# stefanvanberkum/gcnn-cut-selector

Hardware: AMD Instinct MI355X
Metric: bipartite-graph edges/sec (fwd+bwd) per training step, setcov-500 batch=32 (higher is better)
Workload: dtype f32; 1 GPU; setcov-500 rows x batch 32 per GPU (BASELINE configs[1]); step=fwd + mse + bwd + adam, launch=eager, problem=setcov, batch_per_gpu=32, global_batch=32, n_cons=16000, n_vars=32000, n_cuts=1893, n_cons_edges=800000, n_cut_edges=199704, parallelism=dp1

## Files before the change

### gcnn-cut-selector_amd/csrc/k_rows.hpp

```cpp
#pragma once
#include "gcnn_common.hpp"

__device__ __forceinline__ f32x4 mfma16(float a, float b, f32x4 c) {
    return __builtin_amdgcn_mfma_f32_16x16x4f32(a, b, c, 0, 0, 0);
}

struct RTile { float v[4][4]; };

__device__ __forceinline__ const float* lds_here(const float* p) {
    int zero = 0;
    asm volatile("" : "+v"(zero));
    return p + zero;
}

__device__ __forceinline__ void rt_zero(RTile& t) {
#pragma unroll
    for (int m = 0; m < 4; ++m)
#pragma unroll
        for (int i = 0; i < 4; ++i) t.v[m][i] = 0.f;
}
__device__ __forceinline__ void rt_load(RTile& t, const float* x, int row, bool ok, int g) {
#pragma unroll
    for (int m = 0; m < 4; ++m) {
        float4 f = make_float4(0.f, 0.f, 0.f, 0.f);
        if (ok) f = *(const float4*)(x + (size_t)row * EMB + 16 * m + 4 * g);
        t.v[m][0] = f.x; t.v[m][1] = f.y; t.v[m][2] = f.z; t.v[m][3] = f.w;
    }
}
template <int ST = ST_PLAIN>
__device__ __forceinline__ void rt_store(const RTile& t, float* x, int row, bool ok, int g) {
    if (!ok || !x) return;
#pragma unroll
    for (int m = 0; m < 4; ++m) store16<ST>(x + (size_t)row * EMB + 16 * m + 4 * g, t.v[m][0], t.v[m][1], t.v[m][2], t.v[m][3]);
}
enum { GEMM_FWD = 0, GEMM_BWD = 1, GEMM_FWD_RM = 2 };
template <int MODE>
__device__ __forceinline__ void rt_gemm(const RTile& t, float scale, const float* wl, f32x4 (&acc)[4], int lane) {
    const int m = lane & 15, g = lane >> 4;
    wl = lds_here(wl);
#pragma unroll
    for (int mt = 0; mt < 4; ++mt) {
        float av[4][4];
        if (MODE == GEMM_BWD) {
#pragma unroll
            for (int mo = 0; mo < 4; ++mo) {
                const float4 w4 = *(const float4*)(wl + (16 * mo + m) * LDW + 16 * mt + 4 * g);
                av[mo][0] = w4.x; av[mo][1] = w4.y; av[mo][2] = w4.z; av[mo][3] = w4.w;
            }
        } else if (MODE == GEMM_FWD) {
// ... 51 lines not shown
            const float v = o.v[m][i] + bv[i];
            o.v[m][i] = RELU ? fmaxf(v, 0.f) : v;
        }
    }
}
__device__ __forceinline__ void rt_mask(RTile& o, const RTile& act) {
#pragma unroll
    for (int m = 0; m < 4; ++m)
#pragma unroll
        for (int i = 0; i < 4; ++i) o.v[m][i] = act.v[m][i] > 0.f ? o.v[m][i] : 0.f;
}
typedef unsigned short mask16;
__device__ __forceinline__ unsigned rt_mask_bits(const RTile& t) {
    unsigned b = 0;
#pragma unroll
    for (int m = 0; m < 4; ++m)
#pragma unroll
        for (int i = 0; i < 4; ++i) b |= (t.v[m][i] > 0.f ? 1u : 0u) << (4 * m + i);
    return b;
}
__device__ __forceinline__ void rt_mask_store(const RTile& t, mask16* dst, int row, bool ok, int g) {
    if (ok && dst) dst[(size_t)row * 4 + g] = (mask16)rt_mask_bits(t);
}
__device__ __forceinline__ unsigned rt_mask_load(const mask16* src, int row, bool ok, int g) {
    return ok ? (unsigned)src[(size_t)row * 4 + g] : 0u;
}
__device__ __forceinline__ void rt_mask_apply(RTile& o, unsigned bits) {
#pragma unroll
    for (int m = 0; m < 4; ++m)
#pragma unroll
        for (int i = 0; i < 4; ++i) o.v[m][i] = (bits >> (4 * m + i)) & 1u ? o.v[m][i] : 0.f;
}
__device__ __forceinline__ void rt_clear_unless(RTile& o, bool ok) {
#pragma unroll
    for (int m = 0; m < 4; ++m)
#pragma unroll
        for (int i = 0; i < 4; ++i) o.v[m][i] = ok ? o.v[m][i] : 0.f;
}

template <int NM, int NV, int NT, bool K4 = false>
__device__ __forceinline__ void stage_lds(float* smem, const float* const (&w)[NM], const float* const (&v)[NV]) {
    constexpr int PER = 1024 / NT;
    float4 tmp[NM][PER];
    float vec[NV];
    if (K4) {
#pragma unroll
        for (int wi = 0; wi < NM; ++wi)
#pragma unroll
// ... 22 lines not shown
                *(float4*)(smem + wi * 64 * LDW + (idx >> 4) * LDW + (idx & 15) * 4) = tmp[wi][i];
            }
        }
    if (threadIdx.x < 64) {
#pragma unroll
        for (int vi = 0; vi < NV; ++vi) smem[NM * 64 * LDW + vi * 64 + threadIdx.x] = vec[vi];
    }
}
#define ROWS_LDS_FLOATS(NM, NV) ((NM) * 64 * LDW + (NV) * 64)

struct EmbArgs {
    const float *x, *shift, *scale, *w1, *b1; mask16* m_e1;
    const float *w2, *b2; float* xo; mask16* m_x;
    const float* wp[2]; const float* bp[2]; float* po[2];
    int n;
};
template <int F, int NPROJ, int NT, int ST = ST_PLAIN>
__device__ __forceinline__ void emb_program(const EmbArgs& a, float* smem, int bid, int nblk) {
    constexpr int NWAVES = NT / 64, NM = 1 + NPROJ, NV = 2 + NPROJ;
    const int lane = threadIdx.x & 63, wv = threadIdx.x >> 6, j = lane & 15, g = lane >> 4;
    const int ntile = (a.n + 15) >> 4;
    float* vecs = smem + NM * 64 * LDW;
    float* w1s = smem + ROWS_LDS_FLOATS(NM, NV);
    int tile = bid + nblk * wv;
    float xv[F], xn_[F];
    auto load_ops = [&](float (&dst)[F], int t) {
        const int row = t * 16 + j;
#pragma unroll
        for (int f = 0; f < F; ++f) dst[f] = row < a.n ? a.x[(size_t)row * F + f] : 0.f;
    };
    load_ops(xv, tile);
    constexpr int W1N = (F * 64 + NT - 1) / NT;
    float w1r[W1N];
#pragma unroll
    for (int q = 0; q < W1N; ++q) { const int i = threadIdx.x + q * NT; w1r[q] = i < F * 64 ? a.w1[i] : 0.f; }
    if (NPROJ == 2) {
        const float* const w[3] = {a.w2, a.wp[0], a.wp[1]};
        const float* const v[4] = {a.b1, a.b2, a.bp[0], a.bp[1]};
        stage_lds<3, 4, NT, true>((float*)smem, w, v);
    } else {
        const float* const w[2] = {a.w2, a.wp[0]};
        const float* const v[3] = {a.b1, a.b2, a.bp[0]};
        stage_lds<2, 3, NT, true>((float*)smem, w, v);
    }
#pragma unroll
    for (int q = 0; q < W1N; ++q) { const int i = threadIdx.x + q * NT; if (i < F * 64) w1s[i] = w1r[q]; }
    float shift[F], scale[F];
#pragma unroll
    for (int f = 0; f < F; ++f) { shift[f] = a.shift[f]; scale[f] = a.scale[f]; }
    __syncthreads();
    for (; tile < ntile; tile += nblk * NWAVES) {
        load_ops(xn_, tile + nblk * NWAVES);
        const int row = tile * 16 + j;
        const bool ok = row < a.n;
        RTile o, t;
        rt_zero(o);
        const float* w1h = lds_here(w1s);
#pragma unroll
        for (int f = 0; f < F; ++f) {
            const float xn = ok ? (xv[f] + shift[f]) * scale[f] : 0.f;
#pragma unroll
            for (int m = 0; m < 4; ++m) {
                const float4 w = *(const float4*)(w1h + f * EMB + 16 * m + 4 * g);
                o.v[m][0] = fmaf(xn, w.x, o.v[m][0]); o.v[m][1] = fmaf(xn, w.y, o.v[m][1]);
                o.v[m][2] = fmaf(xn, w.z, o.v[m][2]); o.v[m][3] = fmaf(xn, w.w, o.v[m][3]);
            }
        }
        rt_bias<true>(o, vecs, g);
        rt_clear_unless(o, ok);
        rt_mask_store(o, a.m_e1, row, ok, g);
        rt_mm<false>(t, o, 1.f, smem, lane);
        rt_bias<true>(t, vecs + 64, g);
        rt_clear_unless(t, ok);
        rt_store<ST>(t, a.xo, row, ok, g);
        rt_mask_store(t, a.m_x, row, ok, g);
#pragma unroll
        for (int k = 0; k < NPROJ; ++k) {
            rt_mm<false>(o, t, 1.f, smem + (1 + k) * 64 * LDW, lane);
            rt_bias<false>(o, vecs + (2 + k) * 64, g);
            rt_store<ST>(o, a.po[k], row, ok, g);
        }
#pragma unroll
        for (int f = 0; f < F; ++f) xv[f] = xn_[f];
    }
}
#define FUSE_WF (EMB * EMB + EMB)
#define FUSE_W1A (FUSE_WF + EMB * EMB)
#define FUSE_BF (FUSE_W1A + EMB * EMB)
#define FUSE_FLOATS (FUSE_BF + EMB)
struct FuseArgs { const float *wf[3], *bf[3], *s2[3], *w1a[3]; float* out[3]; };
__device__ __forceinline__ void fuse_weights(const FuseArgs& f, const int k, float* smem) {
    float* wfs = smem;
    float* was = smem + 64 * LDW;
    const int t = threadIdx.x;
    if (t < 256) {
        for (int q = t; q < 1024; q += 256) {
            const float4 a = *(const float4*)(f.wf[k] + q * 4), b = *(const float4*)(f.w1a[k] + q * 4);
            *(float4*)(wfs + (q >> 4) * LDW + (q & 15) * 4) = a;
            *(float4*)(was + (q >> 4) * LDW + (q & 15) * 4) = b;
            *(float4*)(f.out[k] + FUSE_WF + q * 4) = a;
            *(float4*)(f.out[k] + FUSE_W1A + q * 4) = b;
        }
        if (t < EMB) f.out[k][FUSE_BF + t] = f.bf[k][t];
    }
    __syncthreads();
    if (t >= 256) return;
// ... 49 lines not shown
    const float* targets; float loss_scale; float* g_o1; float* head_partial;
    int n;
};
enum { CF_PROJ = 0, CF_READOUT = 1, CF_LOSS = 2 };
#define HEAD_SLAB (2 * EMB)
__device__ __forceinline__ float row_sum16(float x) {
    x += __builtin_bit_cast(float, __builtin_amdgcn_update_dpp(0, __builtin_bit_cast(int, x), 0x121, 0xf, 0xf, false));
    x += __builtin_bit_cast(float, __builtin_amdgcn_update_dpp(0, __builtin_bit_cast(int, x), 0x122, 0xf, 0xf, false));
    x += __builtin_bit_cast(float, __builtin_amdgcn_update_dpp(0, __builtin_bit_cast(int, x), 0x124, 0xf, 0xf, false));
    x += __builtin_bit_cast(float, __builtin_amdgcn_update_dpp(0, __builtin_bit_cast(int, x), 0x128, 0xf, 0xf, false));
    return x;
}
__device__ __forceinline__ float readout_score(const RTile& o1, const float* ws_lds, float bs, int g) {
    float sum = 0.f;
    const float* wsv = lds_here(ws_lds);
#pragma unroll
    for (int m = 0; m < 4; ++m) {
        const float4 w = *(const float4*)(wsv + 16 * m + 4 * g);
        sum = fmaf(o1.v[m][0], w.x, fmaf(o1.v[m][1], w.y, fmaf(o1.v[m][2], w.z, fmaf(o1.v[m][3], w.w, sum))));
    }
    sum += __shfl_xor(sum, 16); sum += __shfl_xor(sum, 32);
    return sum + bs;
}
__device__ __forceinline__ void loss_head_tile(RTile& go, const RTile& o1, float score, const ConvFArgs& a, const float* ws_lds,
                                               int tile, int row, bool ok, int lane) {
    const int j = lane & 15, g = lane >> 4;
    const float dlt = ok ? score - a.targets[row] : 0.f;
    const float ds = 2.f * dlt * a.loss_scale;
    const float* wsv = lds_here(ws_lds);
    float* slab = a.head_partial + (size_t)tile * HEAD_SLAB;
#pragma unroll
    for (int m = 0; m < 4; ++m) {
        const float4 w = *(const float4*)(wsv + 16 * m + 4 * g);
        const float wv4[4] = {w.x, w.y, w.z, w.w};
        float cs[4];
#pragma unroll
        for (int i = 0; i < 4; ++i) {
            go.v[m][i] = o1.v[m][i] > 0.f ? ds * wv4[i] : 0.f;
            cs[i] = row_sum16(ds * o1.v[m][i]);
        }
        if (j == 0) *(float4*)(slab + 16 * m + 4 * g) = make_float4(cs[0], cs[1], cs[2], cs[3]);
    }
    const float dbs = row_sum16(ds), ls = row_sum16(a.loss_scale * dlt * dlt);
    if (lane == 0) { slab[EMB] = dbs; slab[EMB + 1] = ls; }
}
template <int TAIL, int NT, bool KEEP_A = false, int ST = ST_PLAIN>
__device__ __forceinline__ void convf_program(const ConvFArgs& a, float* smem, int bid, int nblk) {
    constexpr int NWAVES = NT / 64, NM = KEEP_A ? 5 : 4, NV = 5;
    constexpr int iW1B = NM - 3, iW2 = NM - 2, iWT = NM - 1;
    const int lane = threadIdx.x & 63, wv = threadIdx.x >> 6, j = lane & 15, g = lane >> 4;
    const int ntile = (a.n + 15) >> 4;
    float* vecs = smem + NM * 64 * LDW;
    int tile = bid + nblk * wv;
    struct Ops { RTile s_in, xr; int seg0, seg1; } cur, nxt;
    auto load_ops = [&](Ops& d, int t) {
        const int row = t * 16 + j;
        const bool ok = row < a.n;
        rt_load(d.s_in, a.s, row, ok, g);
        rt_load(d.xr, a.xrecv, row, ok, g);
        d.seg0 = ok ? a.seg_ptr[row] : 0; d.seg1 = ok ? a.seg_ptr[row + 1] : 0;
    };
    load_ops(cur, tile);
    if (KEEP_A) {
        const float* const w[5] = {a.wf, a.w1a, a.w1b, a.w2, a.wt};
        const float* const v[5] = {a.bf, a.b1, a.b2, a.bt, TAIL != CF_PROJ ? a.ws : nullptr};
        stage_lds<5, 5, NT, true>(smem, w, v);
    } else {
        const float* const w[4] = {a.mfuse, a.w1b, a.w2, a.wt};
        const float* const v[5] = {a.ufuse, a.b1, a.b2, a.bt, TAIL != CF_PROJ ? a.ws : nullptr};
        stage_lds<4, 5, NT, true>(smem, w, v);
    }
    const float s2 = KEEP_A ? *a.s2 : 1.f;
    const float bs = TAIL != CF_PROJ ? *a.bs : 0.f;
    __syncthreads();
    for (; tile < ntile; tile += nblk * NWAVES) {
        load_ops(nxt, tile + nblk * NWAVES);
        const RTile &s_in = cur.s_in, &xr = cur.xr;
        const int row = tile * 16 + j;
        const bool ok = row < a.n;
        RTile t0, t1;
        auto add_deg = [&](RTile& t) {
            const float deg = (float)(cur.seg1 - cur.seg0);
            const float* bfv = lds_here(vecs);
#pragma unroll
            for (int m = 0; m < 4; ++m) {
                const float4 b = *(const float4*)(bfv + 16 * m + 4 * g);
                t.v[m][0] = fmaf(deg, b.x, t.v[m][0]); t.v[m][1] = fmaf(deg, b.y, t.v[m][1]);
                t.v[m][2] = fmaf(deg, b.z, t.v[m][2]); t.v[m][3] = fmaf(deg, b.w, t.v[m][3]);
            }
        };
        if (KEEP_A) {
            rt_mm<false>(t0, s_in, 1.f, smem, lane);
            add_deg(t0);
            rt_clear_unless(t0, ok);
            rt_store<ST>(t0, a.a_out, row, ok, g);
            rt_mm2<false>(t1, t0, s2, smem + 64 * LDW, xr, smem + 2 * 64 * LDW, lane);
        } else {
            rt_mm2<false>(t1, s_in, 1.f, smem, xr, smem + iW1B * 64 * LDW, lane);
            add_deg(t1);
        }
        rt_bias<true>(t1, vecs + 64, g);
        rt_clear_unless(t1, ok);
        rt_store<ST>(t1, a.z1, row, ok, g);
        rt_mask_store(t1, a.m_z1, row, ok, g);
        rt_mm<false>(t0, t1, 1.f, smem + iW2 * 64 * LDW, lane);
        rt_bias<true>(t0, vecs + 2 * 64, g);
        rt_clear_unless(t0, ok);
        rt_store<ST>(t0, a.out, row, ok, g);
        rt_mask_store(t0, a.m_out, row, ok, g);
        rt_mm<false>(t1, t0, 1.f, smem + iWT * 64 * LDW, lane);
        if (TAIL == CF_PROJ) {
            rt_bias<false>(t1, vecs + 3 * 64, g);
            rt_store<ST>(t1, a.t_out, row, ok, g);
        } else {
            rt_bias<true>(t1, vecs + 3 * 64, g);
            rt_clear_unless(t1, ok);
            rt_store<ST>(t1, a.t_out, row, ok, g);
            const float score = readout_score(t1, vecs + 4 * 64, bs, g);
            if (g == 0 && ok) a.scores[row] = score;
            if (TAIL == CF_LOSS) {
                RTile go;
                loss_head_tile(go, t1, score, a, vecs + 4 * 64, tile, row, ok, lane);
                rt_store<ST>(go, a.g_o1, row, ok, g);
            }
        }
        cur = nxt;
    }
}
template <int NWAVES, int TAIL, bool KEEP_A = false>
__global__ __launch_bounds__(NWAVES * 64) void k_conv_fwd(ConvFArgs a) {
    extern __shared__ __attribute__((aligned(16))) float smem[];
    convf_program<TAIL, NWAVES * 64, KEEP_A>(a, smem, blockIdx.x, gridDim.x);
}
template <int NWAVES, int TAIL>
__global__ __launch_bounds__(NWAVES * 64) void k_conv_fwd_wt(ConvFArgs a) {
    extern __shared__ __attribute__((aligned(16))) float smem[];
    convf_program<TAIL, NWAVES * 64, false, ST_WT>(a, smem, blockIdx.x, gridDim.x);
}

struct ConvBArgs {
    const float *in, *w0; const mask16* m_out; float* g_out;
    const float* w2; const mask16* m_z1; float* g_z1;
    const float* w1b; float* g_xrecv;
    const float* mfuse; float* g_s;
    const float *s1, *nrows; float* g_precv;
    int n;
};
template <int NT, int ST = ST_PLAIN>
__device__ __forceinline__ void convb_program(const ConvBArgs& a, float* smem, int bid, int nblk) {
    constexpr int NWAVES = NT / 64;
    const int lane = threadIdx.x & 63, wv = threadIdx.x >> 6, j = lane & 15, g = lane >> 4;
    const int ntile = (a.n + 15) >> 4;
    int tile = bid + nblk * wv;
    struct Ops { RTile in, nr; unsigned m0, m1; } cur, nxt;
    auto load_ops = [&](Ops& d, int t) {
        const int row = t * 16 + j;
        const bool ok = row < a.n;
        rt_load(d.in, a.in, row, ok, g);
        d.m0 = rt_mask_load(a.m_out, row, ok, g);
        d.m1 = rt_mask_load(a.m_z1, row, ok, g);
        rt_load(d.nr, a.nrows, row, ok, g);
    };
    load_ops(cur, tile);
    {
        const float* const w[4] = {a.w0, a.w2, a.w1b, a.mfuse};
        const float* const v[1] = {nullptr};
        stage_lds<4, 1, NT>(smem, w, v);
    }
    const float s1 = *a.s1;
    __syncthreads();
    for (; tile < ntile; tile += nblk * NWAVES) {
        load_ops(nxt, tile + nblk * NWAVES);
        const RTile &in = cur.in, &nr = cur.nr;
        const int row = tile * 16 + j;
        const bool ok = row < a.n;
        RTile t0, t1;
        rt_mm<true>(t0, in, 1.f, smem, lane);
        rt_mask_apply(t0, cur.m0);
        rt_store<ST>(t0, a.g_out, row, ok, g);
        rt_mm<true>(t1, t0, 1.f, smem + 64 * LDW, lane);
        rt_mask_apply(t1, cur.m1);
        rt_store<ST>(t1, a.g_z1, row, ok, g);
        rt_mm<true>(t0, t1, 1.f, smem + 2 * 64 * LDW, lane);
        rt_store<ST>(t0, a.g_xrecv, row, ok, g);
        rt_mm<true>(t0, t1, 1.f, smem + 3 * 64 * LDW, lane);
        rt_store<ST>(t0, a.g_s, row, ok, g);
#pragma unroll
        for (int m = 0; m < 4; ++m)
#pragma unroll
            for (int i = 0; i < 4; ++i) t0.v[m][i] = s1 * t0.v[m][i] * nr.v[m][i];
        rt_store<ST>(t0, a.g_precv, row, ok, g);
        cur = nxt;
    }
}

template <int NT>
__device__ __forceinline__ void convturn_program(const ConvFArgs& a, const ConvBArgs& b, float* smem, int bid, int nblk) {
    constexpr int NWAVES = NT / 64, NM = 4;
    const int lane = threadIdx.x & 63, wv = threadIdx.x >> 6, j = lane & 15, g = lane >> 4;
    const int ntile = (a.n + 15) >> 4;
    float* vecs = smem + NM * 64 * LDW;
    int tile = bid + nblk * wv;
    struct Ops { RTile s_in, xr, nr; int seg0, seg1; } cur, nxt;
    auto load_ops = [&](Ops& d, int t) {
        const int row = t * 16 + j;
        const bool ok = row < a.n;
        rt_load(d.s_in, a.s, row, ok, g);
        rt_load(d.xr, a.xrecv, row, ok, g);
        rt_load(d.nr, b.nrows, row, ok, g);
        d.seg0 = ok ? a.seg_ptr[row] : 0; d.seg1 = ok ? a.seg_ptr[row + 1] : 0;
    };
    load_ops(cur, tile);
    {
        const float* const w[4] = {a.mfuse, a.w1b, a.w2, a.wt};
        const float* const v[5] = {a.ufuse, a.b1, a.b2, a.bt, a.ws};
        stage_lds<4, 5, NT>(smem, w, v);
    }
    const float s1 = *b.s1, bs = *a.bs;
    float* const MF = smem; float* const W1B = smem + 64 * LDW;
    float* const W2 = smem + 2 * 64 * LDW; float* const WT = smem + 3 * 64 * LDW;
    __syncthreads();
    for (; tile < ntile; tile += nblk * NWAVES) {
        load_ops(nxt, tile + nblk * NWAVES);
        const int row = tile * 16 + j;
        const bool ok = row < a.n;
        RTile t0, z1, xo, t1;
        rt_mm2<GEMM_FWD_RM>(z1, cur.s_in, 1.f, MF, cur.xr, W1B, lane);
        {
            const float deg = (float)(cur.seg1 - cur.seg0);
            const float* bfv = lds_here(vecs);
#pragma unroll
            for (int m = 0; m < 4; ++m) {
                const float4 bb = *(const float4*)(bfv + 16 * m + 4 * g);
                z1.v[m][0] = fmaf(deg, bb.x, z1.v[m][0]); z1.v[m][1] = fmaf(deg, bb.y, z1.v[m][1]);
                z1.v[m][2] = fmaf(deg, bb.z, z1.v[m][2]); z1.v[m][3] = fmaf(deg, bb.w, z1.v[m][3]);
            }
        }
        rt_bias<true>(z1, vecs + 64, g);
        rt_clear_unless(z1, ok);
        rt_store(z1, a.z1, row, ok, g);
        rt_mm<GEMM_FWD_RM>(xo, z1, 1.f, W2, lane);
        rt_bias<true>(xo, vecs + 2 * 64, g);
        rt_clear_unless(xo, ok);
        rt_store(xo, a.out, row, ok, g);
        rt_mm<GEMM_FWD_RM>(t1, xo, 1.f, WT, lane);
        rt_bias<true>(t1, vecs + 3 * 64, g);
        rt_clear_unless(t1, ok);
        rt_store(t1, a.t_out, row, ok, g);
        const float score = readout_score(t1, vecs + 4 * 64, bs, g);
        if (g == 0 && ok) a.scores[row] = score;
        loss_head_tile(t0, t1, score, a, vecs + 4 * 64, tile, row, ok, lane);
        rt_store(t0, a.g_o1, row, ok, g);
        rt_mm<GEMM_BWD>(t1, t0, 1.f, WT, lane);
        rt_mask(t1, xo);
        rt_store(t1, b.g_out, row, ok, g);
        rt_mm<GEMM_BWD>(t0, t1, 1.f, W2, lane);
        rt_mask(t0, z1);
        rt_store(t0, b.g_z1, row, ok, g);
        rt_mm<GEMM_BWD>(t1, t0, 1.f, W1B, lane);
        rt_store(t1, b.g_xrecv, row, ok, g);
        rt_mm<GEMM_BWD>(t1, t0, 1.f, MF, lane);
        rt_store(t1, b.g_s, row, ok, g);
#pragma unroll
        for (int m = 0; m < 4; ++m)
#pragma unroll
            for (int i = 0; i < 4; ++i) t1.v[m][i] = s1 * t1.v[m][i] * cur.nr.v[m][i];
        rt_store(t1, b.g_precv, row, ok, g);
        cur = nxt;
    }
}
template <int NWAVES>
__global__ __launch_bounds__(NWAVES * 64) void k_conv_turn(ConvFArgs f, ConvBArgs b) {
    extern __shared__ __attribute__((aligned(16))) float smem[];
    convturn_program<NWAVES * 64>(f, b, smem, blockIdx.x, gridDim.x);
}

struct TailBArgs {
    const float *in_a, *wa, *in_b, *wb, *add; const mask16* m_x; float* g_x;
    const float* w2; float* g_e1;
    int n;
};
template <bool HAS_INB, int NT, int ST = ST_PLAIN>
__device__ __forceinline__ void tailb_program(const TailBArgs& a, float* smem, int bid, int nblk) {
    constexpr int NWAVES = NT / 64;
    const int lane = threadIdx.x & 63, wv = threadIdx.x >> 6, j = lane & 15, g = lane >> 4;
    const int ntile = (a.n + 15) >> 4;
    int tile = bid + nblk * wv;
    struct Ops { RTile ia, ib, ad; unsigned mk; } cur, nxt;
    auto load_ops = [&](Ops& d, int t) {
        const int row = t * 16 + j;
        const bool ok = row < a.n;
        rt_load(d.ia, a.in_a, row, ok, g);
        if (HAS_INB) rt_load(d.ib, a.in_b, row, ok, g);
        rt_load(d.ad, a.add, row, ok, g);
        d.mk = rt_mask_load(a.m_x, row, ok, g);
    };
    load_ops(cur, tile);
    const float* const v[1] = {nullptr};
    if (HAS_INB) { const float* const w[3] = {a.wa, a.w2, a.wb}; stage_lds<3, 1, NT>(smem, w, v); }
    else { const float* const w[2] = {a.wa, a.w2}; stage_lds<2, 1, NT>(smem, w, v); }
    __syncthreads();
    for (; tile < ntile; tile += nblk * NWAVES) {
        load_ops(nxt, tile + nblk * NWAVES);
        const RTile &ia = cur.ia, &ib = cur.ib, &ad = cur.ad;
        const int row = tile * 16 + j;
        const bool ok = row < a.n;
        RTile t0, t1;
        if (HAS_INB) rt_mm2<true>(t0, ia, 1.f, smem, ib, smem + 2 * 64 * LDW, lane);
        else rt_mm<true>(t0, ia, 1.f, smem, lane);
#pragma unroll
        for (int m = 0; m < 4; ++m)
#pragma unroll
            for (int i = 0; i < 4; ++i) t0.v[m][i] += ad.v[m][i];
        rt_mask_apply(t0, cur.mk);
        rt_store<ST>(t0, a.g_x, row, ok, g);
        rt_mm<true>(t1, t0, 1.f, smem + 64 * LDW, lane);
        rt_store<ST>(t1, a.g_e1, row, ok, g);
        cur = nxt;
    }
}

struct ConvBGroupArgs { int blk0[3]; ConvBArgs cb; TailBArgs tail; };
template <int NWAVES, int ST = ST_PLAIN>
__device__ __forceinline__ void conv_bwd_body(const ConvBGroupArgs& m, float* smem, const int b) {
    if (b < m.blk0[1]) convb_program<NWAVES * 64, ST>(m.cb, smem, b, m.blk0[1]);
    else tailb_program<false, NWAVES * 64, ST>(m.tail, smem, b - m.blk0[1], m.blk0[2] - m.blk0[1]);
}
template <int NWAVES>
__global__ __launch_bounds__(NWAVES * 64) void k_conv_bwd(ConvBGroupArgs m) {
    extern __shared__ __attribute__((aligned(16))) float smem[];
    conv_bwd_body<NWAVES>(m, smem, blockIdx.x);
}
template <int NWAVES>
__global__ __launch_bounds__(NWAVES * 64) void k_conv_bwd_wt(ConvBGroupArgs m) {
    extern __shared__ __attribute__((aligned(16))) float smem[];
    conv_bwd_body<NWAVES, ST_WT>(m, smem, blockIdx.x);
}
struct TailGroupArgs { int blk0[3]; TailBArgs a, b; };
template <int NWAVES, int ST = ST_PLAIN>
__device__ __forceinline__ void tail_bwd_body(const TailGroupArgs& m, float* smem, const int b) {
    if (b < m.blk0[1]) tailb_program<true, NWAVES * 64, ST>(m.a, smem, b, m.blk0[1]);
// ... 13 lines not shown
```

### gcnn-cut-selector_amd/csrc/k_rows_split.hpp

```cpp
#pragma once
#include "k_rows.hpp"

#define SX_ROW 68
#define SX_FLOATS (2 * 16 * SX_ROW)
struct RQuart { float v[4]; };

struct SplitLane {
    int lane, wv, j, g, phase;
    float* xbuf;
    __device__ __forceinline__ SplitLane(float* exchange) : lane(threadIdx.x & 63), wv(threadIdx.x >> 6), j(lane & 15), g(lane >> 4), phase(0), xbuf(exchange) {}
};

template <int MODE>
__device__ __forceinline__ void rq_gemm(const RTile& t, float scale, const float* wl, f32x4& acc, const SplitLane& L) {
    const int m = L.j, g = L.g, mo = L.wv;
    wl = lds_here(wl);
#pragma unroll
    for (int mt = 0; mt < 4; ++mt) {
        float av[4];
        if (MODE == GEMM_BWD) {
            const float4 w4 = *(const float4*)(wl + (16 * mo + m) * LDW + 16 * mt + 4 * g);
            av[0] = w4.x; av[1] = w4.y; av[2] = w4.z; av[3] = w4.w;
        } else if (MODE == GEMM_FWD) {
            const float4 w4 = *(const float4*)(wl + ((4 * mt + g) * 64 + 16 * mo + m) * 4);
// ... 16 lines not shown
template <int MODE>
__device__ __forceinline__ void rq_mm2(RQuart& o, const RTile& a, float sa, const float* wa, const RTile& b, const float* wb, const SplitLane& L) {
    f32x4 acc = {0.f, 0.f, 0.f, 0.f};
    rq_gemm<MODE>(a, sa, wa, acc, L);
    rq_gemm<MODE>(b, 1.f, wb, acc, L);
#pragma unroll
    for (int i = 0; i < 4; ++i) o.v[i] = acc[i];
}
template <bool RELU>
__device__ __forceinline__ void rq_bias(RQuart& o, const float* vec, const SplitLane& L) {
    const float4 b = *(const float4*)(lds_here(vec) + 16 * L.wv + 4 * L.g);
    const float bv[4] = {b.x, b.y, b.z, b.w};
#pragma unroll
    for (int i = 0; i < 4; ++i) { const float v = o.v[i] + bv[i]; o.v[i] = RELU ? fmaxf(v, 0.f) : v; }
}
__device__ __forceinline__ void rq_clear_unless(RQuart& o, bool ok) {
#pragma unroll
    for (int i = 0; i < 4; ++i) o.v[i] = ok ? o.v[i] : 0.f;
}
__device__ __forceinline__ void rq_mask(RQuart& o, const RQuart& act) {
#pragma unroll
    for (int i = 0; i < 4; ++i) o.v[i] = act.v[i] > 0.f ? o.v[i] : 0.f;
}
__device__ __forceinline__ void rq_load(RQuart& q, const float* x, int row, bool ok, const SplitLane& L) {
    float4 f = make_float4(0.f, 0.f, 0.f, 0.f);
    if (ok) f = *(const float4*)(x + (size_t)row * EMB + 16 * L.wv + 4 * L.g);
    q.v[0] = f.x; q.v[1] = f.y; q.v[2] = f.z; q.v[3] = f.w;
}
__device__ __forceinline__ void rq_store(const RQuart& q, float* x, int row, bool ok, const SplitLane& L) {
    if (!ok || !x) return;
    *(float4*)(x + (size_t)row * EMB + 16 * L.wv + 4 * L.g) = make_float4(q.v[0], q.v[1], q.v[2], q.v[3]);
}
__device__ __forceinline__ void rq_exchange(RTile& full, const RQuart& q, SplitLane& L) {
    float* b = L.xbuf + L.phase * 16 * SX_ROW;
    *(float4*)(b + L.j * SX_ROW + 16 * L.wv + 4 * L.g) = make_float4(q.v[0], q.v[1], q.v[2], q.v[3]);
    __syncthreads();
#pragma unroll
    for (int mt = 0; mt < 4; ++mt) {
        const float4 f = *(const float4*)(b + L.j * SX_ROW + 16 * mt + 4 * L.g);
        full.v[mt][0] = f.x; full.v[mt][1] = f.y; full.v[mt][2] = f.z; full.v[mt][3] = f.w;
    }
    L.phase ^= 1;
}

template <int F, int NPROJ>
__device__ __forceinline__ void emb_split(const EmbArgs& a, float* smem, int bid, int nblk) {
    constexpr int NT = 256, NM = 1 + NPROJ, NV = 2 + NPROJ;
    const int ntile = (a.n + 15) >> 4;
    float* vecs = smem + NM * 64 * LDW;
    float* w1s = smem + ROWS_LDS_FLOATS(NM, NV);
    SplitLane L(smem + EMB_LDS_FLOATS);
    if (NPROJ == 2) {
        const float* const w[3] = {a.w2, a.wp[0], a.wp[1]};
        const float* const v[4] = {a.b1, a.b2, a.bp[0], a.bp[1]};
        stage_lds<3, 4, NT, true>((float*)smem, w, v);
    } else {
        const float* const w[2] = {a.w2, a.wp[0]};
        const float* const v[3] = {a.b1, a.b2, a.bp[0]};
        stage_lds<2, 3, NT, true>((float*)smem, w, v);
    }
    for (int i = threadIdx.x; i < F * 64; i += NT) w1s[i] = a.w1[i];
    float shift[F], scale[F];
#pragma unroll
    for (int f = 0; f < F; ++f) { shift[f] = a.shift[f]; scale[f] = a.scale[f]; }
    __syncthreads();
    for (int tile = bid; tile < ntile; tile += nblk) {
        const int row = tile * 16 + L.j;
        const bool ok = row < a.n;
        RQuart q;
        RTile full, t;
#pragma unroll
        for (int i = 0; i < 4; ++i) q.v[i] = 0.f;
        const float* w1h = lds_here(w1s);
#pragma unroll
        for (int f = 0; f < F; ++f) {
            const float xn = ok ? (a.x[(size_t)row * F + f] + shift[f]) * scale[f] : 0.f;
            const float4 w = *(const float4*)(w1h + f * EMB + 16 * L.wv + 4 * L.g);
            q.v[0] = fmaf(xn, w.x, q.v[0]); q.v[1] = fmaf(xn, w.y, q.v[1]); q.v[2] = fmaf(xn, w.z, q.v[2]); q.v[3] = fmaf(xn, w.w, q.v[3]);
        }
        rq_bias<true>(q, vecs, L);
        rq_clear_unless(q, ok);
        rq_exchange(full, q, L);
        if (L.wv == 0) rt_mask_store(full, a.m_e1, row, ok, L.g);
        rq_mm<GEMM_FWD>(q, full, 1.f, smem, L);
        rq_bias<true>(q, vecs + 64, L);
        rq_clear_unless(q, ok);
        rq_store(q, a.xo, row, ok, L);
        rq_exchange(t, q, L);
        if (L.wv == 0) rt_mask_store(t, a.m_x, row, ok, L.g);
#pragma unroll
        for (int k = 0; k < NPROJ; ++k) {
            rq_mm<GEMM_FWD>(q, t, 1.f, smem + (1 + k) * 64 * LDW, L);
            rq_bias<false>(q, vecs + (2 + k) * 64, L);
            rq_store(q, a.po[k], row, ok, L);
        }
    }
}

template <int TAIL, bool KEEP_A = false>
__device__ __forceinline__ void convf_split(const ConvFArgs& a, float* smem, int bid, int nblk) {
    static_assert(TAIL == CF_PROJ || TAIL == CF_READOUT, "the loss tail runs in convturn_split");
    constexpr int NT = 256, NM = KEEP_A ? 5 : 4;
    constexpr int iW1B = NM - 3, iW2 = NM - 2, iWT = NM - 1;
    const int ntile = (a.n + 15) >> 4;
    float* vecs = smem + NM * 64 * LDW;
    SplitLane L(smem + ROWS_LDS_FLOATS(5, 5));
    if (KEEP_A) {
        const float* const w[5] = {a.wf, a.w1a, a.w1b, a.w2, a.wt};
        const float* const v[5] = {a.bf, a.b1, a.b2, a.bt, TAIL != CF_PROJ ? a.ws : nullptr};
        stage_lds<5, 5, NT, true>(smem, w, v);
    } else {
        const float* const w[4] = {a.mfuse, a.w1b, a.w2, a.wt};
        const float* const v[5] = {a.ufuse, a.b1, a.b2, a.bt, TAIL != CF_PROJ ? a.ws : nullptr};
        stage_lds<4, 5, NT, true>(smem, w, v);
    }
    const float s2 = KEEP_A ? *a.s2 : 1.f;
    const float bs = TAIL != CF_PROJ ? *a.bs : 0.f;
    __syncthreads();
    for (int tile = bid; tile < ntile; tile += nblk) {
        const int row = tile * 16 + L.j;
        const bool ok = row < a.n;
        RTile s_in, xr, full, z;
        rt_load(s_in, a.s, row, ok, L.g);
        rt_load(xr, a.xrecv, row, ok, L.g);
        const float deg = ok ? (float)(a.seg_ptr[row + 1] - a.seg_ptr[row]) : 0.f;
        RQuart q;
        auto add_deg = [&](RQuart& t) {
            const float4 b = *(const float4*)(lds_here(vecs) + 16 * L.wv + 4 * L.g);
            t.v[0] = fmaf(deg, b.x, t.v[0]); t.v[1] = fmaf(deg, b.y, t.v[1]); t.v[2] = fmaf(deg, b.z, t.v[2]); t.v[3] = fmaf(deg, b.w, t.v[3]);
        };
        if (KEEP_A) {
            rq_mm<GEMM_FWD>(q, s_in, 1.f, smem, L);
            add_deg(q);
            rq_clear_unless(q, ok);
            rq_store(q, a.a_out, row, ok, L);
            rq_exchange(full, q, L);
            rq_mm2<GEMM_FWD>(q, full, s2, smem + 64 * LDW, xr, smem + 2 * 64 * LDW, L);
        } else {
            rq_mm2<GEMM_FWD>(q, s_in, 1.f, smem, xr, smem + iW1B * 64 * LDW, L);
            add_deg(q);
        }
        rq_bias<true>(q, vecs + 64, L);
        rq_clear_unless(q, ok);
        rq_store(q, a.z1, row, ok, L);
        rq_exchange(z, q, L);
        if (L.wv == 0) rt_mask_store(z, a.m_z1, row, ok, L.g);
        rq_mm<GEMM_FWD>(q, z, 1.f, smem + iW2 * 64 * LDW, L);
        rq_bias<true>(q, vecs + 2 * 64, L);
// ... 13 lines not shown
            if (L.wv == 0) {
                const float score = readout_score(full, vecs + 4 * 64, bs, L.g);
                if (L.g == 0 && ok) a.scores[row] = score;
            }
        }
    }
}

__device__ __forceinline__ void convturn_split(const ConvFArgs& a, const ConvBArgs& b, float* smem, int bid, int nblk) {
    constexpr int NT = 256, NM = 4;
    const int ntile = (a.n + 15) >> 4;
    float* vecs = smem + NM * 64 * LDW;
    SplitLane L(smem + ROWS_LDS_FLOATS(5, 5));
    {
        const float* const w[4] = {a.mfuse, a.w1b, a.w2, a.wt};
        const float* const v[5] = {a.ufuse, a.b1, a.b2, a.bt, a.ws};
        stage_lds<4, 5, NT>(smem, w, v);
    }
    const float s1 = *b.s1, bs = *a.bs;
    float* const MF = smem; float* const W1B = smem + 64 * LDW;
    float* const W2 = smem + 2 * 64 * LDW; float* const WT = smem + 3 * 64 * LDW;
    __syncthreads();
    for (int tile = bid; tile < ntile; tile += nblk) {
        const int row = tile * 16 + L.j;
        const bool ok = row < a.n;
        RTile s_in, xr, full, o1;
        RQuart nr, q, z1q, xoq;
        rt_load(s_in, a.s, row, ok, L.g);
        rt_load(xr, a.xrecv, row, ok, L.g);
        rq_load(nr, b.nrows, row, ok, L);
        const float deg = ok ? (float)(a.seg_ptr[row + 1] - a.seg_ptr[row]) : 0.f;
        rq_mm2<GEMM_FWD_RM>(z1q, s_in, 1.f, MF, xr, W1B, L);
        {
            const float4 bb = *(const float4*)(lds_here(vecs) + 16 * L.wv + 4 * L.g);
            z1q.v[0] = fmaf(deg, bb.x, z1q.v[0]); z1q.v[1] = fmaf(deg, bb.y, z1q.v[1]); z1q.v[2] = fmaf(deg, bb.z, z1q.v[2]); z1q.v[3] = fmaf(deg, bb.w, z1q.v[3]);
        }
        rq_bias<true>(z1q, vecs + 64, L);
        rq_clear_unless(z1q, ok);
        rq_store(z1q, a.z1, row, ok, L);
        rq_exchange(full, z1q, L);
        rq_mm<GEMM_FWD_RM>(xoq, full, 1.f, W2, L);
        rq_bias<true>(xoq, vecs + 2 * 64, L);
        rq_clear_unless(xoq, ok);
        rq_store(xoq, a.out, row, ok, L);
        rq_exchange(full, xoq, L);
        rq_mm<GEMM_FWD_RM>(q, full, 1.f, WT, L);
        rq_bias<true>(q, vecs + 3 * 64, L);
        rq_clear_unless(q, ok);
        rq_store(q, a.t_out, row, ok, L);
        rq_exchange(o1, q, L);
        const float score = readout_score(o1, vecs + 4 * 64, bs, L.g);
        RTile go;
        if (L.wv == 0) {
            if (L.g == 0 && ok) a.scores[row] = score;
            loss_head_tile(go, o1, score, a, vecs + 4 * 64, tile, row, ok, L.lane);
            rt_store(go, a.g_o1, row, ok, L.g);
        } else {
            const float ds = ok ? 2.f * (score - a.targets[row]) * a.loss_scale : 0.f;
            const float* wsv = lds_here(vecs + 4 * 64);
#pragma unroll
            for (int m = 0; m < 4; ++m) {
                const float4 w = *(const float4*)(wsv + 16 * m + 4 * L.g);
                const float wv4[4] = {w.x, w.y, w.z, w.w};
#pragma unroll
                for (int i = 0; i < 4; ++i) go.v[m][i] = o1.v[m][i] > 0.f ? ds * wv4[i] : 0.f;
            }
        }
        rq_mm<GEMM_BWD>(q, go, 1.f, WT, L);
        rq_mask(q, xoq);
        rq_store(q, b.g_out, row, ok, L);
        rq_exchange(full, q, L);
        rq_mm<GEMM_BWD>(q, full, 1.f, W2, L);
        rq_mask(q, z1q);
        rq_store(q, b.g_z1, row, ok, L);
        rq_exchange(full, q, L);
        rq_mm<GEMM_BWD>(q, full, 1.f, W1B, L);
        rq_store(q, b.g_xrecv, row, ok, L);
        rq_mm<GEMM_BWD>(q, full, 1.f, MF, L);
        rq_store(q, b.g_s, row, ok, L);
#pragma unroll
        for (int i = 0; i < 4; ++i) q.v[i] = s1 * q.v[i] * nr.v[i];
// ... 25 lines not shown
```

Before: 4.091 billion edges/s.

## Clamp row loads and pin next-tile prefetch arrival before stores

Row loads now clamp out-of-range rows to the last valid row, so they are unconditional and branch-free instead of predicated zero-fills. Next-tile prefetches are scoped per iteration and guarded by a 'more' flag. Empty asm 'arrive' barriers force the prefetched registers to be consumed before particular stores (earlier for write-through stores), which controls where the compiler places vmcnt waits so the prefetch latency overlaps compute. Targets are also prefetched alongside other operands, and the wave index is made uniform via readfirstlane. The cost is higher register pressure and compiler-scheduling fragility.

```diff
diff --git a/gcnn-cut-selector_amd/csrc/k_rows.hpp b/gcnn-cut-selector_amd/csrc/k_rows.hpp
--- a/gcnn-cut-selector_amd/csrc/k_rows.hpp
+++ b/gcnn-cut-selector_amd/csrc/k_rows.hpp
@@ -19,12 +19,31 @@
 #pragma unroll
         for (int i = 0; i < 4; ++i) t.v[m][i] = 0.f;
 }
-__device__ __forceinline__ void rt_load(RTile& t, const float* x, int row, bool ok, int g) {
+__device__ __forceinline__ int rt_row(int row, int n) { return row < n ? row : n - 1; }
+__device__ __forceinline__ void rt_load(RTile& t, const float* x, int row, int g) {
 #pragma unroll
     for (int m = 0; m < 4; ++m) {
-        float4 f = make_float4(0.f, 0.f, 0.f, 0.f);
-        if (ok) f = *(const float4*)(x + (size_t)row * EMB + 16 * m + 4 * g);
+        const float4 f = *(const float4*)(x + (size_t)row * EMB + 16 * m + 4 * g);
         t.v[m][0] = f.x; t.v[m][1] = f.y; t.v[m][2] = f.z; t.v[m][3] = f.w;
+    }
+}
+#ifdef GCNN_STORE_PLAIN
+#define RT_ARRIVE_EARLY(ST) false
+#else
+#define RT_ARRIVE_EARLY(ST) ((ST) == ST_WT)
+#endif
+__device__ __forceinline__ int tile_first(int bid, int nblk) {
+    return bid + nblk * __builtin_amdgcn_readfirstlane((int)(threadIdx.x >> 6));
+}
+__device__ __forceinline__ void rt_arrive(float& x) { asm volatile("" : "+v"(x)); }
+__device__ __forceinline__ void rt_arrive(int& x) { asm volatile("" : "+v"(x)); }
+__device__ __forceinline__ void rt_arrive(unsigned& x) { asm volatile("" : "+v"(x)); }
+__device__ __forceinline__ void rt_arrive(RTile& t) {
+#pragma unroll
+    for (int m = 0; m < 4; ++m) {
+        f32x4 q = {t.v[m][0], t.v[m][1], t.v[m][2], t.v[m][3]};
+        asm volatile("" : "+v"(q));
+        t.v[m][0] = q[0]; t.v[m][1] = q[1]; t.v[m][2] = q[2]; t.v[m][3] = q[3];
     }
 }
 template <int ST = ST_PLAIN>
@@ -122,8 +141,8 @@
 __device__ __forceinline__ void rt_mask_store(const RTile& t, mask16* dst, int row, bool ok, int g) {
     if (ok && dst) dst[(size_t)row * 4 + g] = (mask16)rt_mask_bits(t);
 }
-__device__ __forceinline__ unsigned rt_mask_load(const mask16* src, int row, bool ok, int g) {
-    return ok ? (unsigned)src[(size_t)row * 4 + g] : 0u;
+__device__ __forceinline__ unsigned rt_mask_load(const mask16* src, int row, int g) {
+    return (unsigned)src[(size_t)row * 4 + g];
 }
 __device__ __forceinline__ void rt_mask_apply(RTile& o, unsigned bits) {
 #pragma unroll
@@ -192,14 +211,17 @@
     const int ntile = (a.n + 15) >> 4;
     float* vecs = smem + NM * 64 * LDW;
     float* w1s = smem + ROWS_LDS_FLOATS(NM, NV);
-    int tile = bid + nblk * wv;
-    float xv[F], xn_[F];
+    int tile = tile_first(bid, nblk);
+    float xv[F];
     auto load_ops = [&](float (&dst)[F], int t) {
-        const int row = t * 16 + j;
-#pragma unroll
-        for (int f = 0; f < F; ++f) dst[f] = row < a.n ? a.x[(size_t)row * F + f] : 0.f;
+        const int row = rt_row(t * 16 + j, a.n);
+#pragma unroll
+        for (int f = 0; f < F; ++f) dst[f] = a.x[(size_t)row * F + f];
     };
-    load_ops(xv, tile);
+    if (tile < ntile) load_ops(xv, tile);
+    float shift[F], scale[F];
+#pragma unroll
+    for (int f = 0; f < F; ++f) { shift[f] = a.shift[f]; scale[f] = a.scale[f]; }
     constexpr int W1N = (F * 64 + NT - 1) / NT;
     float w1r[W1N];
 #pragma unroll
@@ -215,12 +237,11 @@
     }
 #pragma unroll
     for (int q = 0; q < W1N; ++q) { const int i = threadIdx.x + q * NT; if (i < F * 64) w1s[i] = w1r[q]; }
-    float shift[F], scale[F];
-#pragma unroll
-    for (int f = 0; f < F; ++f) { shift[f] = a.shift[f]; scale[f] = a.scale[f]; }
     __syncthreads();
     for (; tile < ntile; tile += nblk * NWAVES) {
-        load_ops(xn_, tile + nblk * NWAVES);
+        const bool more = tile + nblk * NWAVES < ntile;
+        float xn_[F];
+        if (more) load_ops(xn_, tile + nblk * NWAVES);
         const int row = tile * 16 + j;
         const bool ok = row < a.n;
         RTile o, t;
@@ -242,16 +263,26 @@
         rt_mm<false>(t, o, 1.f, smem, lane);
         rt_bias<true>(t, vecs + 64, g);
         rt_clear_unless(t, ok);
+        if (RT_ARRIVE_EARLY(ST)) {
+#pragma unroll
+            for (int f = 0; f < F; ++f) rt_arrive(xn_[f]);
+        }
         rt_store<ST>(t, a.xo, row, ok, g);
         rt_mask_store(t, a.m_x, row, ok, g);
 #pragma unroll
         for (int k = 0; k < NPROJ; ++k) {
             rt_mm<false>(o, t, 1.f, smem + (1 + k) * 64 * LDW, lane);
             rt_bias<false>(o, vecs + (2 + k) * 64, g);
+            if (!RT_ARRIVE_EARLY(ST) && k == NPROJ - 1) {
+#pragma unroll
+                for (int f = 0; f < F; ++f) rt_arrive(xn_[f]);
+            }
             rt_store<ST>(o, a.po[k], row, ok, g);
         }
-#pragma unroll
-        for (int f = 0; f < F; ++f) xv[f] = xn_[f];
+        if (more) {
+#pragma unroll
+            for (int f = 0; f < F; ++f) xv[f] = xn_[f];
+        }
     }
 }
 #define FUSE_WF (EMB * EMB + EMB)
@@ -347,10 +378,10 @@
     sum += __shfl_xor(sum, 16); sum += __shfl_xor(sum, 32);
     return sum + bs;
 }
-__device__ __forceinline__ void loss_head_tile(RTile& go, const RTile& o1, float score, const ConvFArgs& a, const float* ws_lds,
-                                               int tile, int row, bool ok, int lane) {
+__device__ __forceinline__ void loss_head_tile(RTile& go, const RTile& o1, float score, float target, const ConvFArgs& a, const float* ws_lds,
+                                               int tile, bool ok, int lane) {
     const int j = lane & 15, g = lane >> 4;
-    const float dlt = ok ? score - a.targets[row] : 0.f;
+    const float dlt = ok ? score - target : 0.f;
     const float ds = 2.f * dlt * a.loss_scale;
     const float* wsv = lds_here(ws_lds);
     float* slab = a.head_partial + (size_t)tile * HEAD_SLAB;
@@ -376,16 +407,17 @@
     const int lane = threadIdx.x & 63, wv = threadIdx.x >> 6, j = lane & 15, g = lane >> 4;
     const int ntile = (a.n + 15) >> 4;
     float* vecs = smem + NM * 64 * LDW;
-    int tile = bid + nblk * wv;
-    struct Ops { RTile s_in, xr; int seg0, seg1; } cur, nxt;
+    int tile = tile_first(bid, nblk);
+    struct Ops { RTile s_in, xr; int seg0, seg1; float y; } cur;
     auto load_ops = [&](Ops& d, int t) {
-        const int row = t * 16 + j;
-        const bool ok = row < a.n;
-        rt_load(d.s_in, a.s, row, ok, g);
-        rt_load(d.xr, a.xrecv, row, ok, g);
-        d.seg0 = ok ? a.seg_ptr[row] : 0; d.seg1 = ok ? a.seg_ptr[row + 1] : 0;
+        const int row = rt_row(t * 16 + j, a.n);
+        rt_load(d.s_in, a.s, row, g);
+        rt_load(d.xr, a.xrecv, row, g);
+        d.seg0 = a.seg_ptr[row]; d.seg1 = a.seg_ptr[row + 1];
+        if (TAIL == CF_LOSS) d.y = a.targets[row];
     };
-    load_ops(cur, tile);
+    auto arrive = [&](Ops& d) { rt_arrive(d.s_in); rt_arrive(d.xr); rt_arrive(d.seg0); rt_arrive(d.seg1); if (TAIL == CF_LOSS) rt_arrive(d.y); };
+    if (tile < ntile) load_ops(cur, tile);
     if (KEEP_A) {
         const float* const w[5] = {a.wf, a.w1a, a.w1b, a.w2, a.wt};
         const float* const v[5] = {a.bf, a.b1, a.b2, a.bt, TAIL != CF_PROJ ? a.ws : nullptr};
@@ -399,7 +431,9 @@
     const float bs = TAIL != CF_PROJ ? *a.bs : 0.f;
     __syncthreads();
     for (; tile < ntile; tile += nblk * NWAVES) {
-        load_ops(nxt, tile + nblk * NWAVES);
+        const bool more = tile + nblk * NWAVES < ntile;
+        Ops nxt;
+        if (more) load_ops(nxt, tile + nblk * NWAVES);
         const RTile &s_in = cur.s_in, &xr = cur.xr;
         const int row = tile * 16 + j;
         const bool ok = row < a.n;
@@ -418,6 +452,7 @@
             rt_mm<false>(t0, s_in, 1.f, smem, lane);
             add_deg(t0);
             rt_clear_unless(t0, ok);
+            if (RT_ARRIVE_EARLY(ST)) arrive(nxt);
             rt_store<ST>(t0, a.a_out, row, ok, g);
             rt_mm2<false>(t1, t0, s2, smem + 64 * LDW, xr, smem + 2 * 64 * LDW, lane);
         } else {
@@ -426,6 +461,7 @@
         }
         rt_bias<true>(t1, vecs + 64, g);
         rt_clear_unless(t1, ok);
+        if (RT_ARRIVE_EARLY(ST) && !KEEP_A) arrive(nxt);
         rt_store<ST>(t1, a.z1, row, ok, g);
         rt_mask_store(t1, a.m_z1, row, ok, g);
         rt_mm<false>(t0, t1, 1.f, smem + iW2 * 64 * LDW, lane);
@@ -436,20 +472,22 @@
         rt_mm<false>(t1, t0, 1.f, smem + iWT * 64 * LDW, lane);
         if (TAIL == CF_PROJ) {
             rt_bias<false>(t1, vecs + 3 * 64, g);
+            if (!RT_ARRIVE_EARLY(ST)) arrive(nxt);
             rt_store<ST>(t1, a.t_out, row, ok, g);
         } else {
             rt_bias<true>(t1, vecs + 3 * 64, g);
             rt_clear_unless(t1, ok);
+            if (!RT_ARRIVE_EARLY(ST)) arrive(nxt);
             rt_store<ST>(t1, a.t_out, row, ok, g);
             const float score = readout_score(t1, vecs + 4 * 64, bs, g);
             if (g == 0 && ok) a.scores[row] = score;
             if (TAIL == CF_LOSS) {
                 RTile go;
-                loss_head_tile(go, t1, score, a, vecs + 4 * 64, tile, row, ok, lane);
+                loss_head_tile(go, t1, score, cur.y, a, vecs + 4 * 64, tile, ok, lane);
                 rt_store<ST>(go, a.g_o1, row, ok, g);
             }
         }
-        cur = nxt;
+        if (more) cur = nxt;
     }
 }
 template <int NWAVES, int TAIL, bool KEEP_A = false>
@@ -476,17 +514,17 @@
     constexpr int NWAVES = NT / 64;
     const int lane = threadIdx.x & 63, wv = threadIdx.x >> 6, j = lane & 15, g = lane >> 4;
     const int ntile = (a.n + 15) >> 4;
-    int tile = bid + nblk * wv;
-    struct Ops { RTile in, nr; unsigned m0, m1; } cur, nxt;
+    int tile = tile_first(bid, nblk);
+    struct Ops { RTile in, nr; unsigned m0, m1; } cur;
     auto load_ops = [&](Ops& d, int t) {
-        const int row = t * 16 + j;
-        const bool ok = row < a.n;
-        rt_load(d.in, a.in, row, ok, g);
-        d.m0 = rt_mask_load(a.m_out, row, ok, g);
-        d.m1 = rt_mask_load(a.m_z1, row, ok, g);
-        rt_load(d.nr, a.nrows, row, ok, g);
+        const int row = rt_row(t * 16 + j, a.n);
+        rt_load(d.in, a.in, row, g);
+        d.m0 = rt_mask_load(a.m_out, row, g);
+        d.m1 = rt_mask_load(a.m_z1, row, g);
+        rt_load(d.nr, a.nrows, row, g);
     };
-    load_ops(cur, tile);
+    auto arrive = [&](Ops& d) { rt_arrive(d.in); rt_arrive(d.m0); rt_arrive(d.m1); rt_arrive(d.nr); };
+    if (tile < ntile) load_ops(cur, tile);
     {
         const float* const w[4] = {a.w0, a.w2, a.w1b, a.mfuse};
         const float* const v[1] = {nullptr};
@@ -495,13 +533,16 @@
     const float s1 = *a.s1;
     __syncthreads();
     for (; tile < ntile; tile += nblk * NWAVES) {
-        load_ops(nxt, tile + nblk * NWAVES);
+        const bool more = tile + nblk * NWAVES < ntile;
+        Ops nxt;
+        if (more) load_ops(nxt, tile + nblk * NWAVES);
         const RTile &in = cur.in, &nr = cur.nr;
         const int row = tile * 16 + j;
         const bool ok = row < a.n;
         RTile t0, t1;
         rt_mm<true>(t0, in, 1.f, smem, lane);
         rt_mask_apply(t0, cur.m0);
+        if (RT_ARRIVE_EARLY(ST)) arrive(nxt);
         rt_store<ST>(t0, a.g_out, row, ok, g);
         rt_mm<true>(t1, t0, 1.f, smem + 64 * LDW, lane);
         rt_mask_apply(t1, cur.m1);
@@ -509,13 +550,14 @@
         rt_mm<true>(t0, t1, 1.f, smem + 2 * 64 * LDW, lane);
         rt_store<ST>(t0, a.g_xrecv, row, ok, g);
         rt_mm<true>(t0, t1, 1.f, smem + 3 * 64 * LDW, lane);
+        if (!RT_ARRIVE_EARLY(ST)) arrive(nxt);
         rt_store<ST>(t0, a.g_s, row, ok, g);
 #pragma unroll
         for (int m = 0; m < 4; ++m)
 #pragma unroll
             for (int i = 0; i < 4; ++i) t0.v[m][i] = s1 * t0.v[m][i] * nr.v[m][i];
         rt_store<ST>(t0, a.g_precv, row, ok, g);
-        cur = nxt;
+        if (more) cur = nxt;
     }
 }
 
@@ -525,17 +567,18 @@
     const int lane = threadIdx.x & 63, wv = threadIdx.x >> 6, j = lane & 15, g = lane >> 4;
     const int ntile = (a.n + 15) >> 4;
     float* vecs = smem + NM * 64 * LDW;
-    int tile = bid + nblk * wv;
-    struct Ops { RTile s_in, xr, nr; int seg0, seg1; } cur, nxt;
+    int tile = tile_first(bid, nblk);
+    struct Ops { RTile s_in, xr, nr; int seg0, seg1; float y; } cur;
     auto load_ops = [&](Ops& d, int t) {
-        const int row = t * 16 + j;
-        const bool ok = row < a.n;
-        rt_load(d.s_in, a.s, row, ok, g);
-        rt_load(d.xr, a.xrecv, row, ok, g);
-        rt_load(d.nr, b.nrows, row, ok, g);
-        d.seg0 = ok ? a.seg_ptr[row] : 0; d.seg1 = ok ? a.seg_ptr[row + 1] : 0;
+        const int row = rt_row(t * 16 + j, a.n);
+        rt_load(d.s_in, a.s, row, g);
+        rt_load(d.xr, a.xrecv, row, g);
+        rt_load(d.nr, b.nrows, row, g);
+        d.seg0 = a.seg_ptr[row]; d.seg1 = a.seg_ptr[row + 1];
+        d.y = a.targets[row];
     };
-    load_ops(cur, tile);
+    auto arrive = [&](Ops& d) { rt_arrive(d.s_in); rt_arrive(d.xr); rt_arrive(d.nr); rt_arrive(d.seg0); rt_arrive(d.seg1); rt_arrive(d.y); };
+    if (tile < ntile) load_ops(cur, tile);
     {
         const float* const w[4] = {a.mfuse, a.w1b, a.w2, a.wt};
         const float* const v[5] = {a.ufuse, a.b1, a.b2, a.bt, a.ws};
@@ -546,7 +589,9 @@
     float* const W2 = smem + 2 * 64 * LDW; float* const WT = smem + 3 * 64 * LDW;
     __syncthreads();
     for (; tile < ntile; tile += nblk * NWAVES) {
-        load_ops(nxt, tile + nblk * NWAVES);
+        const bool more = tile + nblk * NWAVES < ntile;
+        Ops nxt;
+        if (more) load_ops(nxt, tile + nblk * NWAVES);
         const int row = tile * 16 + j;
         const bool ok = row < a.n;
         RTile t0, z1, xo, t1;
@@ -574,7 +619,7 @@
         rt_store(t1, a.t_out, row, ok, g);
         const float score = readout_score(t1, vecs + 4 * 64, bs, g);
         if (g == 0 && ok) a.scores[row] = score;
-        loss_head_tile(t0, t1, score, a, vecs + 4 * 64, tile, row, ok, lane);
+        loss_head_tile(t0, t1, score, cur.y, a, vecs + 4 * 64, tile, ok, lane);
         rt_store(t0, a.g_o1, row, ok, g);
         rt_mm<GEMM_BWD>(t1, t0, 1.f, WT, lane);
         rt_mask(t1, xo);
@@ -585,13 +630,14 @@
         rt_mm<GEMM_BWD>(t1, t0, 1.f, W1B, lane);
         rt_store(t1, b.g_xrecv, row, ok, g);
         rt_mm<GEMM_BWD>(t1, t0, 1.f, MF, lane);
+        arrive(nxt);
         rt_store(t1, b.g_s, row, ok, g);
 #pragma unroll
         for (int m = 0; m < 4; ++m)
 #pragma unroll
             for (int i = 0; i < 4; ++i) t1.v[m][i] = s1 * t1.v[m][i] * cur.nr.v[m][i];
         rt_store(t1, b.g_precv, row, ok, g);
-        cur = nxt;
+        if (more) cur = nxt;
     }
 }
 template <int NWAVES>
@@ -610,23 +656,25 @@
     constexpr int NWAVES = NT / 64;
     const int lane = threadIdx.x & 63, wv = threadIdx.x >> 6, j = lane & 15, g = lane >> 4;
     const int ntile = (a.n + 15) >> 4;
-    int tile = bid + nblk * wv;
-    struct Ops { RTile ia, ib, ad; unsigned mk; } cur, nxt;
+    int tile = tile_first(bid, nblk);
+    struct Ops { RTile ia, ib, ad; unsigned mk; } cur;
     auto load_ops = [&](Ops& d, int t) {
-        const int row = t * 16 + j;
-        const bool ok = row < a.n;
-        rt_load(d.ia, a.in_a, row, ok, g);
-        if (HAS_INB) rt_load(d.ib, a.in_b, row, ok, g);
-        rt_load(d.ad, a.add, row, ok, g);
-        d.mk = rt_mask_load(a.m_x, row, ok, g);
+        const int row = rt_row(t * 16 + j, a.n);
+        rt_load(d.ia, a.in_a, row, g);
+        if (HAS_INB) rt_load(d.ib, a.in_b, row, g);
+        rt_load(d.ad, a.add, row, g);
+        d.mk = rt_mask_load(a.m_x, row, g);
     };
-    load_ops(cur, tile);
+    auto arrive = [&](Ops& d) { rt_arrive(d.ia); if (HAS_INB) rt_arrive(d.ib); rt_arrive(d.ad); rt_arrive(d.mk); };
+    if (tile < ntile) load_ops(cur, tile);
     const float* const v[1] = {nullptr};
     if (HAS_INB) { const float* const w[3] = {a.wa, a.w2, a.wb}; stage_lds<3, 1, NT>(smem, w, v); }
     else { const float* const w[2] = {a.wa, a.w2}; stage_lds<2, 1, NT>(smem, w, v); }
     __syncthreads();
     for (; tile < ntile; tile += nblk * NWAVES) {
-        load_ops(nxt, tile + nblk * NWAVES);
+        const bool more = tile + nblk * NWAVES < ntile;
+        Ops nxt;
+        if (more) load_ops(nxt, tile + nblk * NWAVES);
         const RTile &ia = cur.ia, &ib = cur.ib, &ad = cur.ad;
         const int row = tile * 16 + j;
         const bool ok = row < a.n;
@@ -638,10 +686,12 @@
 #pragma unroll
             for (int i = 0; i < 4; ++i) t0.v[m][i] += ad.v[m][i];
         rt_mask_apply(t0, cur.mk);
+        if (RT_ARRIVE_EARLY(ST)) arrive(nxt);
         rt_store<ST>(t0, a.g_x, row, ok, g);
         rt_mm<true>(t1, t0, 1.f, smem + 64 * LDW, lane);
+        if (!RT_ARRIVE_EARLY(ST)) arrive(nxt);
         rt_store<ST>(t1, a.g_e1, row, ok, g);
-        cur = nxt;
+        if (more) cur = nxt;
     }
 }
 
diff --git a/gcnn-cut-selector_amd/csrc/k_rows_split.hpp b/gcnn-cut-selector_amd/csrc/k_rows_split.hpp
--- a/gcnn-cut-selector_amd/csrc/k_rows_split.hpp
+++ b/gcnn-cut-selector_amd/csrc/k_rows_split.hpp
@@ -62,9 +62,8 @@
 #pragma unroll
     for (int i = 0; i < 4; ++i) o.v[i] = act.v[i] > 0.f ? o.v[i] : 0.f;
 }
-__device__ __forceinline__ void rq_load(RQuart& q, const float* x, int row, bool ok, const SplitLane& L) {
-    float4 f = make_float4(0.f, 0.f, 0.f, 0.f);
-    if (ok) f = *(const float4*)(x + (size_t)row * EMB + 16 * L.wv + 4 * L.g);
+__device__ __forceinline__ void rq_load(RQuart& q, const float* x, int row, const SplitLane& L) {
+    const float4 f = *(const float4*)(x + (size_t)row * EMB + 16 * L.wv + 4 * L.g);
     q.v[0] = f.x; q.v[1] = f.y; q.v[2] = f.z; q.v[3] = f.w;
 }
 __device__ __forceinline__ void rq_store(const RQuart& q, float* x, int row, bool ok, const SplitLane& L) {
@@ -105,16 +104,19 @@
     for (int f = 0; f < F; ++f) { shift[f] = a.shift[f]; scale[f] = a.scale[f]; }
     __syncthreads();
     for (int tile = bid; tile < ntile; tile += nblk) {
-        const int row = tile * 16 + L.j;
+        const int row = tile * 16 + L.j, lrow = rt_row(row, a.n);
         const bool ok = row < a.n;
         RQuart q;
         RTile full, t;
+        float xv[F];
+#pragma unroll
+        for (int f = 0; f < F; ++f) xv[f] = a.x[(size_t)lrow * F + f];
 #pragma unroll
         for (int i = 0; i < 4; ++i) q.v[i] = 0.f;
         const float* w1h = lds_here(w1s);
 #pragma unroll
         for (int f = 0; f < F; ++f) {
-            const float xn = ok ? (a.x[(size_t)row * F + f] + shift[f]) * scale[f] : 0.f;
+            const float xn = ok ? (xv[f] + shift[f]) * scale[f] : 0.f;
             const float4 w = *(const float4*)(w1h + f * EMB + 16 * L.wv + 4 * L.g);
             q.v[0] = fmaf(xn, w.x, q.v[0]); q.v[1] = fmaf(xn, w.y, q.v[1]); q.v[2] = fmaf(xn, w.z, q.v[2]); q.v[3] = fmaf(xn, w.w, q.v[3]);
         }
@@ -158,12 +160,12 @@
     const float bs = TAIL != CF_PROJ ? *a.bs : 0.f;
     __syncthreads();
     for (int tile = bid; tile < ntile; tile += nblk) {
-        const int row = tile * 16 + L.j;
+        const int row = tile * 16 + L.j, lrow = rt_row(row, a.n);
         const bool ok = row < a.n;
         RTile s_in, xr, full, z;
-        rt_load(s_in, a.s, row, ok, L.g);
-        rt_load(xr, a.xrecv, row, ok, L.g);
-        const float deg = ok ? (float)(a.seg_ptr[row + 1] - a.seg_ptr[row]) : 0.f;
+        rt_load(s_in, a.s, lrow, L.g);
+        rt_load(xr, a.xrecv, lrow, L.g);
+        const float deg = (float)(a.seg_ptr[lrow + 1] - a.seg_ptr[lrow]);
         RQuart q;
         auto add_deg = [&](RQuart& t) {
             const float4 b = *(const float4*)(lds_here(vecs) + 16 * L.wv + 4 * L.g);
@@ -223,14 +225,15 @@
     float* const W2 = smem + 2 * 64 * LDW; float* const WT = smem + 3 * 64 * LDW;
     __syncthreads();
     for (int tile = bid; tile < ntile; tile += nblk) {
-        const int row = tile * 16 + L.j;
+        const int row = tile * 16 + L.j, lrow = rt_row(row, a.n);
         const bool ok = row < a.n;
         RTile s_in, xr, full, o1;
         RQuart nr, q, z1q, xoq;
-        rt_load(s_in, a.s, row, ok, L.g);
-        rt_load(xr, a.xrecv, row, ok, L.g);
-        rq_load(nr, b.nrows, row, ok, L);
-        const float deg = ok ? (float)(a.seg_ptr[row + 1] - a.seg_ptr[row]) : 0.f;
+        rt_load(s_in, a.s, lrow, L.g);
+        rt_load(xr, a.xrecv, lrow, L.g);
+        rq_load(nr, b.nrows, lrow, L);
+        const float deg = (float)(a.seg_ptr[lrow + 1] - a.seg_ptr[lrow]);
+        const float target = a.targets[lrow];
         rq_mm2<GEMM_FWD_RM>(z1q, s_in, 1.f, MF, xr, W1B, L);
         {
             const float4 bb = *(const float4*)(lds_here(vecs) + 16 * L.wv + 4 * L.g);
@@ -254,10 +257,10 @@
         RTile go;
         if (L.wv == 0) {
             if (L.g == 0 && ok) a.scores[row] = score;
-            loss_head_tile(go, o1, score, a, vecs + 4 * 64, tile, row, ok, L.lane);
+            loss_head_tile(go, o1, score, target, a, vecs + 4 * 64, tile, ok, L.lane);
             rt_store(go, a.g_o1, row, ok, L.g);
         } else {
-            const float ds = ok ? 2.f * (score - a.targets[row]) * a.loss_scale : 0.f;
+            const float ds = ok ? 2.f * (score - target) * a.loss_scale : 0.f;
             const float* wsv = lds_here(vecs + 4 * 64);
 #pragma unroll
             for (int m = 0; m < 4; ++m) {
```

Result: no change. 4.114 billion edges/s (median of 5 runs) (+0.6%).
